# msyriac/orphics

Hardware: AMD Instinct MI355X
Metric: QE kappa reconstructions/sec on 8192^2 maps (higher is better)
Workload: dtype f64

## Files before the change

### orphics_amd/csrc/common.hpp

```cpp
#pragma once
#include <hip/hip_runtime.h>
#include <cstdio>
#include <cstring>
#include <string>
#include "../../include/orphics_amd.h"
#include "cx.hpp"

namespace oa {

std::string& last_error_ref();

inline int fail(const std::string& msg) {
    last_error_ref() = msg;
    return 1;
}

#define OA_HIP(expr)                                                                              \
    do {                                                                                          \
        hipError_t _e = (expr);                                                                   \
        if (_e != hipSuccess)                                                                     \
            return ::oa::fail(std::string(#expr) + ": " + hipGetErrorString(_e) + " (" + __FILE__ + \
                              ":" + std::to_string(__LINE__) + ")");                              \
    } while (0)

// ... 2 lines not shown
        if (!(cond)) return ::oa::fail(std::string(msg)); \
    } while (0)

#define OA_LAUNCH_CHECK() OA_HIP(hipGetLastError())

template <typename T, int N>
struct alignas(sizeof(T) * N > 16 ? 16 : sizeof(T) * N) Arr {
    T v[N];
};

struct DivBinFuse {
    const int32_t* ids; long ipitch;
    const int32_t* ids_t;
    const void* fn_t;
    int tab_logc, tab_rows;
    double pnorm; int nids, nxh;
    double* part;
    long part_cap;
    double* sums;
    unsigned* ticket;
    const int64_t* mcounts; int64_t* n; double* S; double* C;
    int store;
    int gx;
    bool done;
};

inline int flat_grid(long units, int block = 256, int cap = 8192) {
    long g = (units + block - 1) / block;
    if (g < 1) g = 1;
    if (g > cap) g = cap;
// ... 151 lines not shown
```

### orphics_amd/csrc/fft.hip

```cpp
#include <cmath>
#include <vector>
#include "fft_launch.hpp"
#include "fft_r2c_w64.hpp"
#include "fft_r2c_rs4096.hpp"
#include "fft_divbin.hpp"

namespace oa {

template <typename T, int MODE, class SEQ>
__global__ __launch_bounds__(row_maxnt<SEQ>(), waves_per_eu<T>()) void row_fft_kernel(RowArgs<T> a) {
    GpuCtx c{oa_dyn_smem};
    row_fft_body<T, MODE, SEQ>(c, a);
}

#ifndef OA_W64_OCC
#define OA_W64_OCC 1
#endif
__global__ __launch_bounds__(64, OA_W64_OCC) void row_r2c_w64_kernel(RowW64Args a) {
    GpuCtx c{oa_dyn_smem};
    row_r2c_w64_body(c, a);
}

template <typename T, class SEQ, int LR, bool PF>
__global__ __launch_bounds__(row_maxnt<SEQ>(), (sizeof(T) == 8 || PF ? 2 : 3)) void row_r2c_rsplit_kernel(RowArgs<T> a) {
// ... 117 lines not shown
    row_qe8_body<T, A, NZ, LAY, CHAIN>(c, a);
}

template <typename T, class SEQ>
__global__ __launch_bounds__(col_maxnt<SEQ>(), fused_col_waves_per_eu<T>()) void col_div_kernel(ColDivArgs<T> a) {
    GpuCtx c{oa_dyn_smem};
    col_div_body<T, SEQ>(c, a);
}

template <typename T, class SEQ, int LOGC>
__global__ __launch_bounds__((sizeof(T) == 8 ? 512 : 1024), (sizeof(T) == 8 ? 2 : 4)) void col_div_sp_kernel(ColDivArgs<T> a) {
    GpuCtx c{oa_dyn_smem};
    col_div_body<T, SEQ, GpuCtx, LOGC>(c, a);
}

template <typename T, class SEQ, int LOGC>
__global__ __launch_bounds__((sizeof(T) == 8 ? 512 : 1024), (sizeof(T) == 8 ? 2 : 4)) void col_div_sp_bin_kernel(ColDivArgs<T> a, DivBinFuse f) {
    GpuCtx c{oa_dyn_smem};
    col_div_body<T, SEQ, GpuCtx, LOGC, DivBinTail<T>>(c, a, DivBinTail<T>{f});
}

template <typename T, int LOGQ, int LOGC>
__global__ __launch_bounds__((sizeof(T) == 8 ? 384 : 768), (sizeof(T) == 8 ? 2 : 3)) void col_div3_sp_kernel(ColDivArgs<T> a) {
    GpuCtx c{oa_dyn_smem};
    col_div3_body<T, LOGQ, LOGC>(c, a);
}
template <typename T, int LOGQ, int LOGC>
__global__ __launch_bounds__((sizeof(T) == 8 ? 384 : 768), (sizeof(T) == 8 ? 2 : 3)) void col_div3_sp_bin_kernel(ColDivArgs<T> a, DivBinFuse f) {
    GpuCtx c{oa_dyn_smem};
    col_div3_body<T, LOGQ, LOGC, GpuCtx, DivBinTail<T>>(c, a, DivBinTail<T>{f});
}

template <typename T, class SEQ>
__global__ __launch_bounds__(col_maxnt<SEQ>(), waves_per_eu<T>()) void col_deriv_kernel(ColDerivArgs<T> a) {
    GpuCtx c{oa_dyn_smem};
    col_deriv_body<T, SEQ>(c, a);
}

template <typename T, class SEQ>
__global__ __launch_bounds__(col_maxnt<SEQ>(), waves_per_eu<T>()) void col_fft_kernel(ColArgs<T> a) {
    GpuCtx c{oa_dyn_smem};
    col_fft_body<T, SEQ>(c, a);
}

template <typename T, class SEQ>
// ... 274 lines not shown
        if (rc) return;
        rc = launch_col_fwdlegs_cg<T>(st, gx, gy, nt, smem, logL, a, gz);
    }
    template <typename T>
    void col_div(int gx, int gy, int nt, size_t smem, int logL, const ColDivArgs<T>& a, int gz = 1) {
        const bool ok = dispatch_seq(logL, [&](auto seq) {
            using S = decltype(seq);
            if constexpr (seq_logl<S>() <= 8) {
                if (nt > col_maxnt<S>()) { if (!rc) rc = fail("fft: column workgroup size exceeds its launch bound"); return; }
                go(col_div_kernel<T, S>, dim3(gx, gy, gz), nt, smem, a);
            } else if (!rc) rc = fail("fft: unsupported column sub-length");
        });
        if (!ok && !rc) rc = fail("fft: unsupported column length");
    }
    DivBinFuse* fuse = nullptr;
    template <class K, typename T>
    void go_fused(K kern, int gx, int gz, int nt, size_t smem, ColDivArgs<T> a) {
        {
            const hipError_t e = ensure_dyn_lds(reinterpret_cast<const void*>(kern), smem);
            if (e != hipSuccess) { rc = fail(std::string("hipFuncSetAttribute: ") + hipGetErrorString(e)); return; }
        }
        fuse->gx = gx;
        if (!fuse->store) a.out = nullptr;
        const bool tabs = fuse->tab_logc == a.logC && fuse->tab_rows == a.ny;
        a.Fn_t = (tabs && a.fn_moff == 0) ? (const T*)fuse->fn_t : nullptr;
        if (!tabs) fuse->ids_t = nullptr;
        hipLaunchKernelGGL(kern, dim3(gx, 1, gz), dim3(nt), smem, st, a, *fuse);
        hipError_t e = hipGetLastError();
        if (e != hipSuccess) rc = fail(std::string("fft launch: ") + hipGetErrorString(e));
        fuse->done = true;
    }
    template <typename T>
    bool col_div_sp(int gx, size_t smem, int logL, const ColDivArgs<T>& a, int gz = 1) {
        if (rc) return true;
        const int lt = Fft2dPlan<T>::div_lt(), nt = (1 << lt) / EPT;
        const bool narrow = lt < (sizeof(T) == 4 ? 14 : 13);
        constexpr int lc11 = sizeof(T) == 4 ? 3 : 2, lc10 = lc11 + 1;
        if (fuse && !a.accumulate && (long)gx * gz * fuse->nids <= fuse->part_cap && (logL == 10 || logL == 11 || (logL == 12 && !narrow)) &&
            (size_t)(nt / 64) * fuse->nids * sizeof(double) <= ((size_t)1 << lt) * sizeof(cx<T>)) {
            if (logL == 12) go_fused(col_div_sp_bin_kernel<T, Seq<16, 16, 16>, lc11 - 1>, gx, gz, nt, smem, a);
            else if (logL == 11 && !narrow) go_fused(col_div_sp_bin_kernel<T, Seq<16, 16, 8>, lc11>, gx, gz, nt, smem, a);
            else if (logL == 10 && !narrow) go_fused(col_div_sp_bin_kernel<T, Seq<16, 16, 4>, lc10>, gx, gz, nt, smem, a);
            else if (logL == 11) go_fused(col_div_sp_bin_kernel<T, Seq<16, 16, 8>, lc11 - 1>, gx, gz, nt, smem, a);
            else go_fused(col_div_sp_bin_kernel<T, Seq<16, 16, 4>, lc10 - 1>, gx, gz, nt, smem, a);
            return true;
        }
        if (logL == 12 && !narrow) { go(col_div_sp_kernel<T, Seq<16, 16, 16>, lc11 - 1>, dim3(gx, 1, gz), nt, smem, a); return true; }
        if (logL == 11 && !narrow) { go(col_div_sp_kernel<T, Seq<16, 16, 8>, lc11>, dim3(gx, 1, gz), nt, smem, a); return true; }
        if (logL == 10 && !narrow) { go(col_div_sp_kernel<T, Seq<16, 16, 4>, lc10>, dim3(gx, 1, gz), nt, smem, a); return true; }
        if (logL == 11) { go(col_div_sp_kernel<T, Seq<16, 16, 8>, lc11 - 1>, dim3(gx, 1, gz), nt, smem, a); return true; }
        if (logL == 10) { go(col_div_sp_kernel<T, Seq<16, 16, 4>, lc10 - 1>, dim3(gx, 1, gz), nt, smem, a); return true; }
        return false;
    }
    template <typename T>
    void col_div3(int gx, size_t smem, int rows, const ColDivArgs<T>& a, int gz = 1) {
        if (rc) return;
        constexpr int lc = sizeof(T) == 4 ? 3 : 2;
        if (rows != 1536 && rows != 768) { rc = fail("fft: unsupported 3 x 2^k divergence grid"); return; }
        const int nt = a.NT;
        if (fuse && !a.accumulate && (long)gx * gz * fuse->nids <= fuse->part_cap &&
            (size_t)(nt / 64) * fuse->nids * sizeof(double) <= ((size_t)rows << a.logC) * sizeof(cx<T>)) {
            if (rows == 1536) go_fused(col_div3_sp_bin_kernel<T, 8, lc>, gx, gz, nt, smem, a);
            else go_fused(col_div3_sp_bin_kernel<T, 7, lc + 1>, gx, gz, nt, smem, a);
            return;
        }
        if (rows == 1536) go(col_div3_sp_kernel<T, 8, lc>, dim3(gx, 1, gz), nt, smem, a);
        else go(col_div3_sp_kernel<T, 7, lc + 1>, dim3(gx, 1, gz), nt, smem, a);
    }
    template <typename T>
    void col_deriv(int gx, int gy, int nt, size_t smem, const ColDerivArgs<T>& a, int nz) {
        const bool ok = dispatch_seq(a.logL, [&](auto seq) {
            using S = decltype(seq);
            if constexpr (seq_logl<S>() <= 8) {
                if (nt > col_maxnt<S>()) { if (!rc) rc = fail("fft: column workgroup size exceeds its launch bound"); return; }
                go(col_deriv_kernel<T, S>, dim3(gx, gy, nz), nt, smem, a);
            } else if (!rc) rc = fail("fft: unsupported column sub-length");
        });
        if (!ok && !rc) rc = fail("fft: unsupported column length");
// ... 722 lines not shown
```

### orphics_amd/csrc/fft_divbin.hpp

```cpp
#pragma once
#include "fft_launch.hpp"

namespace oa {

#if defined(__HIP_DEVICE_COMPILE__) && !(defined(__gfx942__) || defined(__gfx950__))
#error "DivBinTail: the ticket hand-over relies on gfx942 / gfx950 behaviour (agent-scope relaxed atomic stores are sc1 write-through, stores count in vmcnt)"
#endif

template <int CTRL>
__device__ __forceinline__ double dpp_f64(double v) {
    const unsigned long long u = __builtin_bit_cast(unsigned long long, v);
    const int lo = __builtin_amdgcn_update_dpp(0, (int)(unsigned)u, CTRL, 0xf, 0xf, false);
    const int hi = __builtin_amdgcn_update_dpp(0, (int)(unsigned)(u >> 32), CTRL, 0xf, 0xf, false);
    return __builtin_bit_cast(double, ((unsigned long long)(unsigned)hi << 32) | (unsigned long long)(unsigned)lo);
}
__device__ __forceinline__ double readlane_f64(double v, int lane) {
    const unsigned long long u = __builtin_bit_cast(unsigned long long, v);
    const unsigned lo = (unsigned)__builtin_amdgcn_readlane((int)(unsigned)u, lane);
    const unsigned hi = (unsigned)__builtin_amdgcn_readlane((int)(unsigned)(u >> 32), lane);
    return __builtin_bit_cast(double, ((unsigned long long)hi << 32) | (unsigned long long)lo);
}
__device__ __forceinline__ double wave_total_f64(double v) {
    v += dpp_f64<0xB1>(v);
    v += dpp_f64<0x4E>(v);
    v += dpp_f64<0x141>(v);
    v += dpp_f64<0x140>(v);
    return ((readlane_f64(v, 0) + readlane_f64(v, 16)) + readlane_f64(v, 32)) + readlane_f64(v, 48);
}

template <typename T>
struct DivBinTail {
    static constexpr bool active = true;
    DivBinFuse f;
    double* rows = nullptr;

    __device__ __forceinline__ void begin(GpuCtx&, void* lds) {
        rows = reinterpret_cast<double*>(lds);
        const int nw = blockDim.x >> 6;
        for (int i = threadIdx.x; i < nw * f.nids; i += blockDim.x) rows[i] = 0.0;
    }
    __device__ __forceinline__ int id_at(unsigned yfull, int col) const { return f.ids[(long)yfull * f.ipitch + col]; }
    __device__ __forceinline__ bool packed_ids() const { return f.ids_t != nullptr; }
    __device__ __forceinline__ int id_at_t(long i) const { return f.ids_t[i]; }
    __device__ __forceinline__ void add(GpuCtx&, int id, T pw, int col) {
        const int m = (col == 0 || col == f.nxh) ? 1 : (col < f.nxh ? 2 : 0);
        const bool ok = id >= 0 && id < f.nids && m > 0;
        const double v = ok ? (double)(pw * (T)f.pnorm) * (double)m : 0.0;
        const int lane = threadIdx.x & 63;
        double* row = rows + (threadIdx.x >> 6) * f.nids;
        unsigned long long act = __ballot(ok);
        while (act) {
            const int leader = __ffsll((long long)act) - 1;
            const int lid = __shfl(id, leader, 64);
            const bool mine = ok && id == lid;
            const unsigned long long mm = __ballot(mine);
            const double sv = wave_total_f64(mine ? v : 0.0);
            if (lane == leader) row[lid] += sv;
            act &= ~mm;
        }
    }
    __device__ __forceinline__ void finish(GpuCtx&) {
        __shared__ int s_last;
        const int t = threadIdx.x, nt = blockDim.x, nw = nt >> 6, nids = f.nids;
        __syncthreads();
        const long wg = (long)blockIdx.z * gridDim.x + blockIdx.x;
        for (int i = t; i < nids; i += nt) {
            double s = 0.0;
            for (int k = 0; k < nw; ++k) s += rows[k * nids + i];
            __hip_atomic_store(f.part + wg * nids + i, s, __ATOMIC_RELAXED, __HIP_MEMORY_SCOPE_AGENT);
        }
        asm volatile("s_waitcnt vmcnt(0)" ::: "memory");
        __syncthreads();
        if (t == 0)
            s_last = (__hip_atomic_fetch_add(f.ticket, 1u, OA_TICKET_ORDER, __HIP_MEMORY_SCOPE_AGENT) == gridDim.x * gridDim.z - 1) ? 1 : 0;
        __syncthreads();
        if (!s_last) return;
        const int d = nids - 2;
        int NI = 1;
        while (NI < nids && NI < nt) NI <<= 1;
        const int G = nt / NI > 0 ? nt / NI : 1, gi = t / NI, ii = t - gi * NI;
        double* red = rows;
        const int gx = (int)gridDim.x;
        for (int z = 0; z < (int)gridDim.z; ++z) {
            for (int i0 = 0; i0 < nids; i0 += NI) {
                const int i = i0 + ii;
                __syncthreads();
                if (gi < G) {
                    double s = 0.0;
                    if (i < nids) {
                        const double* pz = f.part + ((long)z * gx) * nids + i;
                        int b = gi;
                        for (; b + 3 * G < gx; b += 4 * G) {
                            const double p0 = __hip_atomic_load(pz + (long)b * nids, __ATOMIC_RELAXED, __HIP_MEMORY_SCOPE_AGENT);
                            const double p1 = __hip_atomic_load(pz + (long)(b + G) * nids, __ATOMIC_RELAXED, __HIP_MEMORY_SCOPE_AGENT);
                            const double p2 = __hip_atomic_load(pz + (long)(b + 2 * G) * nids, __ATOMIC_RELAXED, __HIP_MEMORY_SCOPE_AGENT);
                            const double p3 = __hip_atomic_load(pz + (long)(b + 3 * G) * nids, __ATOMIC_RELAXED, __HIP_MEMORY_SCOPE_AGENT);
                            s += (p0 + p1) + (p2 + p3);
                        }
                        for (; b < gx; b += G) s += __hip_atomic_load(pz + (long)b * nids, __ATOMIC_RELAXED, __HIP_MEMORY_SCOPE_AGENT);
                    }
                    red[gi * NI + ii] = s;
                }
                __syncthreads();
                double tot = 0.0;
                if (gi == 0 && i < nids) {
                    for (int k = 0; k < G; ++k) tot += red[k * NI + ii];
                    f.sums[(long)z * nids + i] = tot;
                }
                __syncthreads();
                if (gi == 0 && i >= 1 && i <= d) red[G * NI + i - 1] = tot / (double)f.mcounts[i];
            }
            __syncthreads();
            const double* bv = red + G * NI;
            if (f.S) {
                for (int a = t; a < d; a += nt) f.S[a] += bv[a];
                for (long e = t; e < (long)d * d; e += nt) {
                    const int ra = (int)(e / d), cb = (int)(e - (long)ra * d);
                    f.C[e] += bv[ra] * bv[cb];
                }
            }
        }
        if (t == 0) {
            if (f.n) f.n[0] += (int64_t)gridDim.z;
            __hip_atomic_store(f.ticket, 0u, __ATOMIC_RELAXED, __HIP_MEMORY_SCOPE_AGENT);
        }
    }
};

}
```

### orphics_amd/csrc/fft_kernels.hpp

```cpp
#pragma once
#include <type_traits>
#include "cx.hpp"
#include "philox.hpp"

namespace oa {

constexpr int EPT = 16;
#ifndef OA_COL_LOGC
#define OA_COL_LOGC 5
#endif
constexpr int COL_LOGC = OA_COL_LOGC;

enum RowMode { ROW_R2C = 0, ROW_C2R = 1, ROW_C2C_F = 2, ROW_C2C_I = 3, ROW_WIN = 4 };

template <typename T>
OA_HD cx<T> w16(int k) {
    const T c1 = (T)0.92387953251128673848L;
    const T s1 = (T)0.38268343236508978178L;
    const T h = (T)0.70710678118654752440L;
    switch (k) {
        case 0: return mk<T>((T)1, (T)0);
        case 1: return mk<T>(c1, -s1);
        case 2: return mk<T>(h, -h);
        case 3: return mk<T>(s1, -c1);
// ... 1471 lines not shown
    long pitch;
    long opitch;
    int width, logC, NT;
    const cx<T>* tw;
    int logTw;
    long in_gs, in_ns, out_gs, out_ks;
    int accumulate;
    int rband, ny;
    int yshift;
    long in_moff, out_moff;
    long fn_moff;
    const T* Fn_t;
};

struct NoDivTail {
    static constexpr bool active = false;
    template <class Ctx> OA_HD void begin(Ctx&, void*) {}
    OA_HD int id_at(unsigned, int) const { return -1; }
    OA_HD bool packed_ids() const { return false; }
    OA_HD int id_at_t(long) const { return -1; }
    template <class Ctx, typename T> OA_HD void add(Ctx&, int, T, int) {}
    template <class Ctx> OA_HD void finish(Ctx&) {}
};

template <typename T, class SEQ, class Ctx, int LOGC = COL_LOGC, class Tail = NoDivTail>
OA_HD void col_div_body(Ctx& ctx, const ColDivArgs<T>& a, Tail tail = Tail{}) {
    cx<T>* s = reinterpret_cast<cx<T>*>(ctx.smem());
    constexpr int logL = Log2x<SEQ::r0>::v + Log2x<SEQ::r1>::v + Log2x<SEQ::r2>::v + Log2x<SEQ::r3>::v;
    constexpr int n = SEQ::n;
    constexpr int RL = SEQ::get(n - 1), LRL = Log2x<RL>::v, NB = EPT / RL;
    constexpr int logNs = logL - LRL;
    constexpr int logC = LOGC;
    constexpr int NT = ((1 << (seq_total_log<SEQ>() + LOGC)) / EPT) > 0 ? ((1 << (seq_total_log<SEQ>() + LOGC)) / EPT) : 1;
    const int tid = ctx.tid();
    int tile = ctx.bid_x();
    if ((sizeof(cx<T>) << LOGC) < 128) {
// ... 23 lines not shown
        ctx.sync();
        stage_out<T, R0, false, false>(s, vb, tid, NT, logL, logC, 0, 0, NoStore{});
        ctx.sync();
        stage_in<T, RL, false, false>(s, vb, tid, NT, logL, logC, 0, l0, twl, logL, NoLoad{});
    } else {
        col_pipeline_to_regs<T, SEQ>(ctx, s, va, tid, NT, logC, twl, logL, la);
        ctx.sync();
        col_pipeline_to_regs<T, SEQ>(ctx, s, vb, tid, NT, logC, twl, logL, lb);
    }
    const long oorg = g * a.out_gs * a.opitch + c0;
    const T* Fnb = a.Fn + zmap * a.fn_moff + oorg;
    cx<T>* outb = a.out + omo + oorg;
    const unsigned ostr = (unsigned)(a.out_ks * a.opitch);
    if constexpr (Tail::active) {
        ctx.sync();
        tail.begin(ctx, s);
        ctx.sync();
        T pw[EPT];
        int idv[EPT];
#pragma unroll
        for (int u = 0; u < NB; ++u) {
            const int b = tid + u * NT;
            const int c = b & ((1 << logC) - 1), j = b >> logC;
            const bool cok = c < ncols;
            const int kq = j & ((1 << logNs) - 1);
            const int base = ((j - kq) << LRL) + kq;
            const T lx = cok ? a.lxd[c0 + c] : (T)0;
#pragma unroll
            for (int t = 0; t < RL; ++t) {
                const int k = base + (t << logNs);
                const unsigned y = (unsigned)(g * a.out_gs) + (unsigned)k * (unsigned)a.out_ks;
                const bool ok = cok && !(a.rband && (int)y >= a.rband && (int)y <= a.ny - a.rband);
                const unsigned up = (a.yshift && y >= (unsigned)(a.ny >> 1)) ? (unsigned)a.yshift : 0u;
                const unsigned i = (unsigned)k * ostr + (unsigned)c + up * (unsigned)a.opitch;
                pw[u * RL + t] = (T)0;
                idv[u * RL + t] = -1;
                if (ok) {
                    const long ti_ = (((long)tile << logL) + k) * (1 << logC) + c;
                    const T fn = a.Fn_t ? a.Fn_t[ti_] : Fnb[i];
                    cx<T> d = mul_pi(va[u * RL + t] * lx + vb[u * RL + t] * a.lyd[y + up]) * fn;
                    if (a.out) {
                        if (a.accumulate) d = d + outb[i];
                        outb[i] = d;
                    }
                    pw[u * RL + t] = d.x * d.x + d.y * d.y;
                    idv[u * RL + t] = tail.packed_ids() ? tail.id_at_t((((long)tile << logL) + k) * (1 << logC) + c) : tail.id_at(y + up, c0 + c);
                }
            }
        }
#pragma unroll
        for (int u = 0; u < NB; ++u) {
            const int c = (tid + u * NT) & ((1 << logC) - 1);
#pragma unroll
            for (int t = 0; t < RL; ++t) tail.add(ctx, idv[u * RL + t], pw[u * RL + t], c0 + c);
        }
        tail.finish(ctx);
    } else {
#pragma unroll
    for (int u = 0; u < NB; ++u) {
        const int b = tid + u * NT;
        const int c = b & ((1 << logC) - 1), j = b >> logC;
        if (c >= ncols) continue;
        const int kq = j & ((1 << logNs) - 1);
        const int base = ((j - kq) << LRL) + kq;
        const T lx = a.lxd[c0 + c];
#pragma unroll
        for (int t = 0; t < RL; ++t) {
            const int k = base + (t << logNs);
            const unsigned y = (unsigned)(g * a.out_gs) + (unsigned)k * (unsigned)a.out_ks;
// ... 74 lines not shown
#pragma unroll
            for (int r = 0; r < 6; ++r) x[it][r] = s[((r * Q + pk[it]) << logC) + pc[it]];
            const cx<T> w3 = w1[it] * w2[it], w5 = w4[it] * w1[it];
            x[it][1] = x[it][1] * w1[it]; x[it][2] = x[it][2] * w2[it]; x[it][3] = x[it][3] * w3;
            x[it][4] = x[it][4] * w4[it]; x[it][5] = x[it][5] * w5;
            dft6<T>(x[it]);
        }
    };
    finish(va, xa);
    ctx.sync();
    finish(vb, xb);
    const T* Fnb = a.Fn + zmap * a.fn_moff + c0;
    cx<T>* outb = a.out + omo + c0;
    if constexpr (Tail::active) {
        ctx.sync();
        tail.begin(ctx, s);
        ctx.sync();
        T pw[NIT * 6];
        int idv[NIT * 6];
#pragma unroll
        for (int it = 0; it < NIT; ++it) {
            const int c = pc[it], k = pk[it];
            const bool cok = pv[it] && c < ncols;
            const T lx = cok ? a.lxd[c0 + c] : (T)0;
#pragma unroll
            for (int q = 0; q < 6; ++q) {
                const unsigned y = (unsigned)(k + Q * q);
                const bool ok = cok && !(a.rband && (int)y >= a.rband && (int)y <= a.ny - a.rband);
                const unsigned up = (a.yshift && y >= (unsigned)(N >> 1)) ? (unsigned)a.yshift : 0u;
                const unsigned i = (y + up) * (unsigned)a.opitch + (unsigned)c;
                pw[it * 6 + q] = (T)0;
                idv[it * 6 + q] = -1;
                if (ok) {
                    const long ti_ = ((long)tile * N + y) * C + c;
                    const T fn = a.Fn_t ? a.Fn_t[ti_] : Fnb[i];
                    cx<T> d = mul_pi(xa[it][q] * lx + xb[it][q] * a.lyd[y + up]) * fn;
                    if (a.out) {
                        if (a.accumulate) d = d + outb[i];
                        outb[i] = d;
                    }
                    pw[it * 6 + q] = d.x * d.x + d.y * d.y;
                    idv[it * 6 + q] = tail.packed_ids() ? tail.id_at_t(ti_) : tail.id_at(y + up, c0 + c);
                }
            }
        }
#pragma unroll
        for (int it = 0; it < NIT; ++it) {
#pragma unroll
            for (int q = 0; q < 6; ++q) tail.add(ctx, idv[it * 6 + q], pw[it * 6 + q], c0 + pc[it]);
        }
        tail.finish(ctx);
    } else {
#pragma unroll
        for (int it = 0; it < NIT; ++it) {
            const int c = pc[it], k = pk[it];
            if (!pv[it] || c >= ncols) continue;
            const T lx = a.lxd[c0 + c];
#pragma unroll
            for (int q = 0; q < 6; ++q) {
                const unsigned y = (unsigned)(k + Q * q);
                if (a.rband && (int)y >= a.rband && (int)y <= a.ny - a.rband) continue;
                const unsigned up = (a.yshift && y >= (unsigned)(N >> 1)) ? (unsigned)a.yshift : 0u;
                const unsigned i = (y + up) * (unsigned)a.opitch + (unsigned)c;
                cx<T> d = mul_pi(xa[it][q] * lx + xb[it][q] * a.lyd[y + up]) * Fnb[i];
// ... 442 lines not shown
```

### orphics_amd/csrc/pipeline.hip

```cpp
#include <dlfcn.h>
#include <cstdlib>
#include <algorithm>
#include <functional>
#include <string>
#include <utility>
#include <vector>
#include "common.hpp"
#include "fft_plan.hpp"

namespace oa {

constexpr int MC_BATCH_MAX = 6;

struct DevBuf {
    void* p = nullptr;
    size_t bytes = 0;
    int reserve(size_t need, bool zero = false) {
        if (bytes >= need) return 0;
        if (p) { OA_HIP(hipDeviceSynchronize()); release(); }
        OA_HIP(hipMalloc(&p, need));
        bytes = need;
        if (zero) OA_HIP(hipMemset(p, 0, need));
        return 0;
    }
// ... 32 lines not shown
    DevBuf rdn0_pool;
    unsigned long rdn0_gen = 0;
    int rdn0_my = 0;
    int rdn0_ran_batched = 0;
    DevBuf rdn0mv_legs;
    DevBuf rdn0mv_pool;
    DevBuf n1_pool;
    std::vector<const void*> rdn0mv_key;
    int rdn0mv_band[5] = {0, 0, 0, 0, 0};
    int rdn0mv_my = 0;
    unsigned long rdn0mv_gen = 0;
    struct DivTabs {
        DevBuf fn_t, ids_t;
        unsigned long tab_gen = 0;
        int tab_rows = 0, tab_logc = 0, tab_wk = 0;
    } dt[2];
    DivTabs& tabs_of(int rows) { return (my3 && rows == my3) ? dt[1] : dt[0]; }
    const DivTabs& tabs_of(int rows) const { return (my3 && rows == my3) ? dt[1] : dt[0]; }
    unsigned long bind_gen = 1;
    DevBuf fb_t;
    unsigned long fb_gen = 0;
    int fb_my = 0, fb_wl = 0, fb_rl = 0;
    void** mv_ftab = nullptr;
    std::vector<const void*> mv_fkey;
    int opt_mc_batch = MC_BATCH_MAX;
    bool opt_mv_batch = true;
    bool opt_mv_rowbatch = true;
    bool opt_mv_chain = true;
    bool opt_divbin = true;
    bool opt_win_fused = true;
// ... 50 lines not shown
    return 0;
}

void pipeline_release(oa_plan* p) {
    if (!p || !p->pipe) return;
    Pipeline* q = (Pipeline*)p->pipe;
    if (q->work) (void)hipFree(q->work);
    if (q->bin_scratch) (void)hipFree(q->bin_scratch);
    if (q->sums) (void)hipFree(q->sums);
    if (q->counts_full) (void)hipFree(q->counts_full);
    if (q->counts_tmp) (void)hipFree(q->counts_tmp);
    if (q->ticket) (void)hipFree(q->ticket);
    if (q->mv_ftab) (void)hipFree(q->mv_ftab);
    if (q->mv_rtab) (void)hipFree(q->mv_rtab);
    for (DevBuf* b : {&q->split_legs, &q->mc_src, &q->lens_pool, &q->mvmc, &q->mvwin, &q->rdn0_legs, &q->rdn0_pool, &q->rdn0mv_legs, &q->rdn0mv_pool, &q->n1_pool, &q->dt[0].fn_t, &q->dt[0].ids_t,
                      &q->dt[1].fn_t, &q->dt[1].ids_t, &q->fb_t}) b->release();
    if (q->band) (void)oa_plan_destroy(q->band);
    q->release_band();
    q->brows.release();
    q->bs_tab.release();
    if (q->pb.plan) (void)oa_plan_destroy(q->pb.plan);
    for (DevBuf* b : {&q->pb.planes, &q->pb.stab, &q->pb.mrows, &q->pb.mwin, &q->pb.mc.pool}) b->release();
    delete q;
    p->pipe = nullptr;
}

static int ensure_work(oa_plan* p, Pipeline* q) {
    if (q->work) return 0;
    const size_t pb = plane_bytes(p);
    OA_HIP(hipMalloc(&q->work, 7 * pb));
    OA_HIP(hipMemset(q->work, 0, 7 * pb));
// ... 233 lines not shown
                                                nullptr, q->bin_scratch, 0, 0, stream)
                                 : fail(std::string("oa_plan_set_bins: padded bin ids: ") + hipGetErrorString(e));
        (void)hipStreamSynchronize((hipStream_t)stream);
        (void)hipFree(ids4);
        if (z4) (void)hipFree(z4);
        if (rc) return rc;
    }
    if (p->mixed) return (q->FG && q->band) ? mixed_bins(p, q, (hipStream_t)stream) : 0;
    return ensure_div_tables(p, q, (hipStream_t)stream);
}

void* oa_plan_kappa(oa_plan* p) { return (p && p->pipe) ? ((Pipeline*)p->pipe)->kk : nullptr; }
const int64_t* oa_plan_bin_counts(oa_plan* p) { return (p && p->pipe) ? ((Pipeline*)p->pipe)->counts_full : nullptr; }

static bool divbin_enabled(const Pipeline* q) { return q->opt_divbin; }
static int ensure_div_tables(oa_plan* p, Pipeline* q, hipStream_t st, int rows) {
    Pipeline::DivTabs* const t = &q->tabs_of(rows);
    if (!(q->Fn && q->ids && (rows == 1024 || rows == 2048 || rows == 4096 || (q->my3 && rows == q->my3)) && q->wk > 0)) { t->tab_rows = 0; return 0; }
    const int logc = div_tile_logc(p, rows);
    if (t->tab_gen == q->bind_gen && t->tab_rows == rows && t->tab_logc == logc && t->tab_wk == q->wk) return 0;
    const size_t rs = p->dtype == OA_F32 ? 4 : 8;
    const long tiles = ((long)q->wk + (1 << logc) - 1) >> logc, total = (tiles * rows) << logc;
    if (int rc = t->fn_t.reserve((size_t)total * rs)) return rc;
    if (int rc = t->ids_t.reserve((size_t)total * 4)) return rc;
    if (int rc = pack_tiles(p, q->Fn, t->fn_t.p, rows, logc, q->wk, (int)rs, st)) return rc;
    if (int rc = pack_tiles(p, q->ids, t->ids_t.p, rows, logc, q->wk, 4, st)) return rc;
    t->tab_gen = q->bind_gen; t->tab_rows = rows; t->tab_logc = logc; t->tab_wk = q->wk;
    return 0;
}
static int ensure_div_tables(oa_plan* p, Pipeline* q, hipStream_t st) {
    if (int rc = ensure_div_tables(p, q, st, q->my)) return rc;
    return q->my3 ? ensure_div_tables(p, q, st, q->my3) : 0;
}
static const void* fband_table(oa_plan* p, Pipeline* q, hipStream_t st) {
    static const bool off = exp_env("OA_NO_FBAND_TABLE") != nullptr;
    const int my = q->map_grid();
    if (off || !q->FG || my <= 0 || !qe_rsplit_lr(p, my, q->wl, q->wk, q->mrow)) return nullptr;
    if (q->fb_t.p && q->fb_gen == q->bind_gen && q->fb_my == my && q->fb_wl == q->wl && q->fb_rl == q->rl) return q->fb_t.p;
    if (q->fb_t.reserve((size_t)qe_fband_table_entries(p, q->wl, my) * elem_bytes(p))) { (void)hipGetLastError(); return nullptr; }
    if (qe_fband_pack_w(p, q->FG, q->FH, q->fb_t.p, q->wl, q->rl, my, st)) return nullptr;
    q->fb_gen = q->bind_gen; q->fb_my = my; q->fb_wl = q->wl; q->fb_rl = q->rl;
    return q->fb_t.p;
}
static DivBinFuse make_fuse(const oa_plan* p, const Pipeline* q, int64_t* n, double* S, double* C, int store, int rows = -1) {
    DivBinFuse f{};
    if (rows < 0) rows = q->my;
    const Pipeline::DivTabs& t = q->tabs_of(rows);
    if (t.tab_rows && t.tab_gen == q->bind_gen && t.tab_rows == rows && t.tab_wk == q->wk) {
        f.ids_t = (const int32_t*)t.ids_t.p; f.fn_t = t.fn_t.p; f.tab_logc = t.tab_logc; f.tab_rows = t.tab_rows;
    }
    f.ids = q->ids; f.ipitch = p->kp; f.pnorm = q->norm; f.nids = q->nids; f.nxh = p->nx / 2;
    f.part = (double*)q->bin_scratch; f.part_cap = (long)(oa_bin_scratch_bytes(q->nids) / (long)sizeof(double)) * MC_BATCH_MAX;
    f.sums = q->sums; f.ticket = q->ticket; f.mcounts = q->counts_full; f.n = n; f.S = S; f.C = C; f.store = store; f.done = false;
    return f;
}

static int qe_tt_impl(oa_plan* p, const void* real_map, const void* kX, const void* kY, void* out_kappa_hc, int zero_outside,
                      void* stream, DivBinFuse* fuse, int rows_done = 0);
static int qe_mv_pow2(oa_plan* p, Pipeline* q, const MvCall& c, void* out, int accumulate, int leg_cols, int kappa_cols, int leg_rows,
                      int kappa_rows, int mrow, int zero_outside, hipStream_t st, bool keep_planes);
int oa_qe_tt(oa_plan* p, const void* real_map, const void* kX, const void* kY, void* out_kappa_hc, int zero_outside,
             void* stream) {
    if (p && p->mixed) {
        OA_REQUIRE(p->pipe && ((Pipeline*)p->pipe)->FG, "oa_qe_tt: call oa_plan_set_filters first");
// ... 2014 lines not shown
```

Measured before the change: 5971.

## Bin fused column power via precomputed per-tile run-length tables of bin ids

Builds a host-side table of runs of equal bin ids per column tile and uploads it. When the table is present, the fused column-divergence/binning kernel writes power into LDS by position and sums contiguous runs per bin, instead of loading per-element ids and scattering into per-wave bin rows. The aim is to remove the per-element id loads and the scattered LDS accumulation. In exchange the kernel needs more LDS, and table construction adds a blocking device-to-host copy, a host pass and stream syncs whenever the tables are rebuilt.

```diff
diff --git a/orphics_amd/csrc/common.hpp b/orphics_amd/csrc/common.hpp
--- a/orphics_amd/csrc/common.hpp
+++ b/orphics_amd/csrc/common.hpp
@@ -40,6 +40,8 @@
     const int32_t* ids_t;
     const void* fn_t;
     int tab_logc, tab_rows;
+    const unsigned long long* run_ent; const int32_t* run_off;
+    int run_w, run_rb, run_cap;
     double pnorm; int nids, nxh;
     double* part;
     long part_cap;
diff --git a/orphics_amd/csrc/divbin_runs.hpp b/orphics_amd/csrc/divbin_runs.hpp
--- /dev/null
+++ b/orphics_amd/csrc/divbin_runs.hpp
@@ -0,0 +1,65 @@
+#pragma once
+#include <cstddef>
+#include <cstdint>
+#include <vector>
+
+namespace oa {
+
+constexpr int DIVRUN_MAX_LEN = 64;
+
+inline uint64_t divrun_pack(int col, int first, int len, int id) {
+    return (uint64_t)((uint32_t)first | ((uint32_t)len << 16) | ((uint32_t)col << 24)) | ((uint64_t)(uint32_t)id << 32);
+}
+inline int divrun_first(uint64_t e) { return (int)(e & 0xffffu); }
+inline int divrun_len(uint64_t e) { return (int)((e >> 16) & 0xffu); }
+inline int divrun_col(uint64_t e) { return (int)((e >> 24) & 0xffu); }
+inline int divrun_id(uint64_t e) { return (int)(uint32_t)(e >> 32); }
+
+struct DivRunTable {
+    std::vector<uint64_t> ent;
+    std::vector<int32_t> off;
+};
+
+inline bool divbin_build_runs(const int32_t* ids_t, int tiles, int rows, int logc, int width, int rband, int nids, int nxh, int max_entries,
+                              DivRunTable* out) {
+    out->ent.clear();
+    out->off.clear();
+    if (tiles < 1 || rows < 1 || rows > 0x10000 || logc < 0 || logc > 8 || nids < 1) return false;
+    const int C = 1 << logc;
+    out->off.reserve((size_t)tiles * (nids + 1));
+    std::vector<uint64_t> runs;
+    std::vector<int32_t> cnt((size_t)nids + 1);
+    for (int t = 0; t < tiles; ++t) {
+        runs.clear();
+        const int32_t* tid = ids_t + (size_t)t * rows * C;
+        for (int c = 0; c < C; ++c) {
+            const long col = (long)t * C + c;
+            if (col >= width || col > nxh) continue;
+            int first = 0, len = 0, cur = -1;
+            for (int y = 0; y <= rows; ++y) {
+                const bool kept = y < rows && !(rband > 0 && y >= rband && y <= rows - rband);
+                const int id = kept ? tid[(size_t)y * C + c] : -1;
+                const bool valid = id >= 0 && id < nids;
+                if (len > 0 && valid && id == cur && len < DIVRUN_MAX_LEN) { ++len; continue; }
+                if (len > 0) runs.push_back(divrun_pack(c, first, len, cur));
+                len = 0;
+                if (valid) { first = y; len = 1; cur = id; }
+            }
+        }
+        if ((long)runs.size() > (long)max_entries) {
+            out->ent.clear();
+            out->off.clear();
+            return false;
+        }
+        for (int i = 0; i <= nids; ++i) cnt[i] = 0;
+        for (uint64_t e : runs) ++cnt[divrun_id(e) + 1];
+        const int32_t base = (int32_t)out->ent.size();
+        for (int i = 0; i < nids; ++i) cnt[i + 1] += cnt[i];
+        for (int i = 0; i <= nids; ++i) out->off.push_back(base + cnt[i]);
+        out->ent.resize((size_t)base + runs.size());
+        for (uint64_t e : runs) out->ent[(size_t)base + cnt[divrun_id(e)]++] = e;
+    }
+    return true;
+}
+
+}
diff --git a/orphics_amd/csrc/fft.hip b/orphics_amd/csrc/fft.hip
--- a/orphics_amd/csrc/fft.hip
+++ b/orphics_amd/csrc/fft.hip
@@ -1,3 +1,4 @@
+#include <algorithm>
 #include <cmath>
 #include <vector>
 #include "fft_launch.hpp"
@@ -155,10 +156,11 @@
     col_div_body<T, SEQ, GpuCtx, LOGC>(c, a);
 }
 
-template <typename T, class SEQ, int LOGC>
+template <typename T, bool RUNS> using DivTailOf = std::conditional_t<RUNS, DivRunTail<T>, DivBinTail<T>>;
+template <typename T, class SEQ, int LOGC, bool RUNS>
 __global__ __launch_bounds__((sizeof(T) == 8 ? 512 : 1024), (sizeof(T) == 8 ? 2 : 4)) void col_div_sp_bin_kernel(ColDivArgs<T> a, DivBinFuse f) {
     GpuCtx c{oa_dyn_smem};
-    col_div_body<T, SEQ, GpuCtx, LOGC, DivBinTail<T>>(c, a, DivBinTail<T>{f});
+    col_div_body<T, SEQ, GpuCtx, LOGC, DivTailOf<T, RUNS>>(c, a, DivTailOf<T, RUNS>{f});
 }
 
 template <typename T, int LOGQ, int LOGC>
@@ -166,10 +168,10 @@
     GpuCtx c{oa_dyn_smem};
     col_div3_body<T, LOGQ, LOGC>(c, a);
 }
-template <typename T, int LOGQ, int LOGC>
+template <typename T, int LOGQ, int LOGC, bool RUNS>
 __global__ __launch_bounds__((sizeof(T) == 8 ? 384 : 768), (sizeof(T) == 8 ? 2 : 3)) void col_div3_sp_bin_kernel(ColDivArgs<T> a, DivBinFuse f) {
     GpuCtx c{oa_dyn_smem};
-    col_div3_body<T, LOGQ, LOGC, GpuCtx, DivBinTail<T>>(c, a, DivBinTail<T>{f});
+    col_div3_body<T, LOGQ, LOGC, GpuCtx, DivTailOf<T, RUNS>>(c, a, DivTailOf<T, RUNS>{f});
 }
 
 template <typename T, class SEQ>
@@ -474,15 +476,19 @@
         if (!ok && !rc) rc = fail("fft: unsupported column length");
     }
     DivBinFuse* fuse = nullptr;
+#define OA_GO_FUSED(K, ...) go_fused(K<__VA_ARGS__, false>, K<__VA_ARGS__, true>, gx, gz, nt, smem, a)
     template <class K, typename T>
-    void go_fused(K kern, int gx, int gz, int nt, size_t smem, ColDivArgs<T> a) {
+    void go_fused(K kern_ids, K kern_runs, int gx, int gz, int nt, size_t smem, ColDivArgs<T> a) {
+        const bool tabs = fuse->tab_logc == a.logC && fuse->tab_rows == a.ny;
+        const bool runs = tabs && fuse->run_ent && fuse->run_w == a.width && fuse->run_rb == a.rband && fuse->run_cap <= 2 * nt;
+        const K kern = runs ? kern_runs : kern_ids;
+        if (runs) smem = std::max(smem, divrun_lds_bytes(a.ny, a.logC, nt, sizeof(T) == 8));
         {
             const hipError_t e = ensure_dyn_lds(reinterpret_cast<const void*>(kern), smem);
             if (e != hipSuccess) { rc = fail(std::string("hipFuncSetAttribute: ") + hipGetErrorString(e)); return; }
         }
         fuse->gx = gx;
         if (!fuse->store) a.out = nullptr;
-        const bool tabs = fuse->tab_logc == a.logC && fuse->tab_rows == a.ny;
         a.Fn_t = (tabs && a.fn_moff == 0) ? (const T*)fuse->fn_t : nullptr;
         if (!tabs) fuse->ids_t = nullptr;
         hipLaunchKernelGGL(kern, dim3(gx, 1, gz), dim3(nt), smem, st, a, *fuse);
@@ -498,11 +504,11 @@
         constexpr int lc11 = sizeof(T) == 4 ? 3 : 2, lc10 = lc11 + 1;
         if (fuse && !a.accumulate && (long)gx * gz * fuse->nids <= fuse->part_cap && (logL == 10 || logL == 11 || (logL == 12 && !narrow)) &&
             (size_t)(nt / 64) * fuse->nids * sizeof(double) <= ((size_t)1 << lt) * sizeof(cx<T>)) {
-            if (logL == 12) go_fused(col_div_sp_bin_kernel<T, Seq<16, 16, 16>, lc11 - 1>, gx, gz, nt, smem, a);
-            else if (logL == 11 && !narrow) go_fused(col_div_sp_bin_kernel<T, Seq<16, 16, 8>, lc11>, gx, gz, nt, smem, a);
-            else if (logL == 10 && !narrow) go_fused(col_div_sp_bin_kernel<T, Seq<16, 16, 4>, lc10>, gx, gz, nt, smem, a);
-            else if (logL == 11) go_fused(col_div_sp_bin_kernel<T, Seq<16, 16, 8>, lc11 - 1>, gx, gz, nt, smem, a);
-            else go_fused(col_div_sp_bin_kernel<T, Seq<16, 16, 4>, lc10 - 1>, gx, gz, nt, smem, a);
+            if (logL == 12) OA_GO_FUSED(col_div_sp_bin_kernel, T, Seq<16, 16, 16>, lc11 - 1);
+            else if (logL == 11 && !narrow) OA_GO_FUSED(col_div_sp_bin_kernel, T, Seq<16, 16, 8>, lc11);
+            else if (logL == 10 && !narrow) OA_GO_FUSED(col_div_sp_bin_kernel, T, Seq<16, 16, 4>, lc10);
+            else if (logL == 11) OA_GO_FUSED(col_div_sp_bin_kernel, T, Seq<16, 16, 8>, lc11 - 1);
+            else OA_GO_FUSED(col_div_sp_bin_kernel, T, Seq<16, 16, 4>, lc10 - 1);
             return true;
         }
         if (logL == 12 && !narrow) { go(col_div_sp_kernel<T, Seq<16, 16, 16>, lc11 - 1>, dim3(gx, 1, gz), nt, smem, a); return true; }
@@ -520,8 +526,8 @@
         const int nt = a.NT;
         if (fuse && !a.accumulate && (long)gx * gz * fuse->nids <= fuse->part_cap &&
             (size_t)(nt / 64) * fuse->nids * sizeof(double) <= ((size_t)rows << a.logC) * sizeof(cx<T>)) {
-            if (rows == 1536) go_fused(col_div3_sp_bin_kernel<T, 8, lc>, gx, gz, nt, smem, a);
-            else go_fused(col_div3_sp_bin_kernel<T, 7, lc + 1>, gx, gz, nt, smem, a);
+            if (rows == 1536) OA_GO_FUSED(col_div3_sp_bin_kernel, T, 8, lc);
+            else OA_GO_FUSED(col_div3_sp_bin_kernel, T, 7, lc + 1);
             return;
         }
         if (rows == 1536) go(col_div3_sp_kernel<T, 8, lc>, dim3(gx, 1, gz), nt, smem, a);
diff --git a/orphics_amd/csrc/fft_divbin.hpp b/orphics_amd/csrc/fft_divbin.hpp
--- a/orphics_amd/csrc/fft_divbin.hpp
+++ b/orphics_amd/csrc/fft_divbin.hpp
@@ -28,13 +28,78 @@
     return ((readlane_f64(v, 0) + readlane_f64(v, 16)) + readlane_f64(v, 32)) + readlane_f64(v, 48);
 }
 
+template <class Partial>
+__device__ __forceinline__ void divbin_handover(const DivBinFuse& f, double* red, Partial partial) {
+    __shared__ int s_last;
+    const int t = threadIdx.x, nt = blockDim.x, nids = f.nids;
+    const long wg = (long)blockIdx.z * gridDim.x + blockIdx.x;
+    for (int i = t; i < nids; i += nt) {
+        const double s = partial(i);
+        __hip_atomic_store(f.part + wg * nids + i, s, __ATOMIC_RELAXED, __HIP_MEMORY_SCOPE_AGENT);
+    }
+    asm volatile("s_waitcnt vmcnt(0)" ::: "memory");
+    __syncthreads();
+    if (t == 0)
+        s_last = (__hip_atomic_fetch_add(f.ticket, 1u, OA_TICKET_ORDER, __HIP_MEMORY_SCOPE_AGENT) == gridDim.x * gridDim.z - 1) ? 1 : 0;
+    __syncthreads();
+    if (!s_last) return;
+    const int d = nids - 2;
+    int NI = 1;
+    while (NI < nids && NI < nt) NI <<= 1;
+    const int G = nt / NI > 0 ? nt / NI : 1, gi = t / NI, ii = t - gi * NI;
+    const int gx = (int)gridDim.x;
+    for (int z = 0; z < (int)gridDim.z; ++z) {
+        for (int i0 = 0; i0 < nids; i0 += NI) {
+            const int i = i0 + ii;
+            __syncthreads();
+            if (gi < G) {
+                double s = 0.0;
+                if (i < nids) {
+                    const double* pz = f.part + ((long)z * gx) * nids + i;
+                    int b = gi;
+                    for (; b + 3 * G < gx; b += 4 * G) {
+                        const double p0 = __hip_atomic_load(pz + (long)b * nids, __ATOMIC_RELAXED, __HIP_MEMORY_SCOPE_AGENT);
+                        const double p1 = __hip_atomic_load(pz + (long)(b + G) * nids, __ATOMIC_RELAXED, __HIP_MEMORY_SCOPE_AGENT);
+                        const double p2 = __hip_atomic_load(pz + (long)(b + 2 * G) * nids, __ATOMIC_RELAXED, __HIP_MEMORY_SCOPE_AGENT);
+                        const double p3 = __hip_atomic_load(pz + (long)(b + 3 * G) * nids, __ATOMIC_RELAXED, __HIP_MEMORY_SCOPE_AGENT);
+                        s += (p0 + p1) + (p2 + p3);
+                    }
+                    for (; b < gx; b += G) s += __hip_atomic_load(pz + (long)b * nids, __ATOMIC_RELAXED, __HIP_MEMORY_SCOPE_AGENT);
+                }
+                red[gi * NI + ii] = s;
+            }
+            __syncthreads();
+            double tot = 0.0;
+            if (gi == 0 && i < nids) {
+                for (int k = 0; k < G; ++k) tot += red[k * NI + ii];
+                f.sums[(long)z * nids + i] = tot;
+            }
+            __syncthreads();
+            if (gi == 0 && i >= 1 && i <= d) red[G * NI + i - 1] = tot / (double)f.mcounts[i];
+        }
+        __syncthreads();
+        const double* bv = red + G * NI;
+        if (f.S) {
+            for (int a = t; a < d; a += nt) f.S[a] += bv[a];
+            for (long e = t; e < (long)d * d; e += nt) {
+                const int ra = (int)(e / d), cb = (int)(e - (long)ra * d);
+                f.C[e] += bv[ra] * bv[cb];
+            }
+        }
+    }
+    if (t == 0) {
+        if (f.n) f.n[0] += (int64_t)gridDim.z;
+        __hip_atomic_store(f.ticket, 0u, __ATOMIC_RELAXED, __HIP_MEMORY_SCOPE_AGENT);
+    }
+}
+
 template <typename T>
 struct DivBinTail {
-    static constexpr bool active = true;
+    static constexpr bool active = true, needs_ids = true;
     DivBinFuse f;
     double* rows = nullptr;
 
-    __device__ __forceinline__ void begin(GpuCtx&, void* lds) {
+    __device__ __forceinline__ void begin(GpuCtx&, void* lds, int, int, int) {
         rows = reinterpret_cast<double*>(lds);
         const int nw = blockDim.x >> 6;
         for (int i = threadIdx.x; i < nw * f.nids; i += blockDim.x) rows[i] = 0.0;
@@ -42,7 +107,7 @@
     __device__ __forceinline__ int id_at(unsigned yfull, int col) const { return f.ids[(long)yfull * f.ipitch + col]; }
     __device__ __forceinline__ bool packed_ids() const { return f.ids_t != nullptr; }
     __device__ __forceinline__ int id_at_t(long i) const { return f.ids_t[i]; }
-    __device__ __forceinline__ void add(GpuCtx&, int id, T pw, int col) {
+    __device__ __forceinline__ void add(GpuCtx&, int id, T pw, int col, int) {
         const int m = (col == 0 || col == f.nxh) ? 1 : (col < f.nxh ? 2 : 0);
         const bool ok = id >= 0 && id < f.nids && m > 0;
         const double v = ok ? (double)(pw * (T)f.pnorm) * (double)m : 0.0;
@@ -60,71 +125,87 @@
         }
     }
     __device__ __forceinline__ void finish(GpuCtx&) {
-        __shared__ int s_last;
-        const int t = threadIdx.x, nt = blockDim.x, nw = nt >> 6, nids = f.nids;
-        __syncthreads();
-        const long wg = (long)blockIdx.z * gridDim.x + blockIdx.x;
-        for (int i = t; i < nids; i += nt) {
+        const int nw = blockDim.x >> 6, nids = f.nids;
+        const double* r = rows;
+        __syncthreads();
+        divbin_handover(f, rows, [=](int i) {
             double s = 0.0;
-            for (int k = 0; k < nw; ++k) s += rows[k * nids + i];
-            __hip_atomic_store(f.part + wg * nids + i, s, __ATOMIC_RELAXED, __HIP_MEMORY_SCOPE_AGENT);
-        }
-        asm volatile("s_waitcnt vmcnt(0)" ::: "memory");
-        __syncthreads();
-        if (t == 0)
-            s_last = (__hip_atomic_fetch_add(f.ticket, 1u, OA_TICKET_ORDER, __HIP_MEMORY_SCOPE_AGENT) == gridDim.x * gridDim.z - 1) ? 1 : 0;
-        __syncthreads();
-        if (!s_last) return;
-        const int d = nids - 2;
-        int NI = 1;
-        while (NI < nids && NI < nt) NI <<= 1;
-        const int G = nt / NI > 0 ? nt / NI : 1, gi = t / NI, ii = t - gi * NI;
-        double* red = rows;
-        const int gx = (int)gridDim.x;
-        for (int z = 0; z < (int)gridDim.z; ++z) {
-            for (int i0 = 0; i0 < nids; i0 += NI) {
-                const int i = i0 + ii;
-                __syncthreads();
-                if (gi < G) {
-                    double s = 0.0;
-                    if (i < nids) {
-                        const double* pz = f.part + ((long)z * gx) * nids + i;
-                        int b = gi;
-                        for (; b + 3 * G < gx; b += 4 * G) {
-                            const double p0 = __hip_atomic_load(pz + (long)b * nids, __ATOMIC_RELAXED, __HIP_MEMORY_SCOPE_AGENT);
-                            const double p1 = __hip_atomic_load(pz + (long)(b + G) * nids, __ATOMIC_RELAXED, __HIP_MEMORY_SCOPE_AGENT);
-                            const double p2 = __hip_atomic_load(pz + (long)(b + 2 * G) * nids, __ATOMIC_RELAXED, __HIP_MEMORY_SCOPE_AGENT);
-                            const double p3 = __hip_atomic_load(pz + (long)(b + 3 * G) * nids, __ATOMIC_RELAXED, __HIP_MEMORY_SCOPE_AGENT);
-                            s += (p0 + p1) + (p2 + p3);
-                        }
-                        for (; b < gx; b += G) s += __hip_atomic_load(pz + (long)b * nids, __ATOMIC_RELAXED, __HIP_MEMORY_SCOPE_AGENT);
-                    }
-                    red[gi * NI + ii] = s;
-                }
-                __syncthreads();
-                double tot = 0.0;
-                if (gi == 0 && i < nids) {
-                    for (int k = 0; k < G; ++k) tot += red[k * NI + ii];
-                    f.sums[(long)z * nids + i] = tot;
-                }
-                __syncthreads();
-                if (gi == 0 && i >= 1 && i <= d) red[G * NI + i - 1] = tot / (double)f.mcounts[i];
-            }
-            __syncthreads();
-            const double* bv = red + G * NI;
-            if (f.S) {
-                for (int a = t; a < d; a += nt) f.S[a] += bv[a];
-                for (long e = t; e < (long)d * d; e += nt) {
-                    const int ra = (int)(e / d), cb = (int)(e - (long)ra * d);
-                    f.C[e] += bv[ra] * bv[cb];
-                }
-            }
-        }
-        if (t == 0) {
-            if (f.n) f.n[0] += (int64_t)gridDim.z;
-            __hip_atomic_store(f.ticket, 0u, __ATOMIC_RELAXED, __HIP_MEMORY_SCOPE_AGENT);
-        }
+            for (int k = 0; k < nw; ++k) s += r[k * nids + i];
+            return s;
+        });
     }
 };
 
-}
+__host__ __device__ inline int divrun_col_stride(int rows, int logc) {
+    const int want = (32 >> logc) > 0 ? (32 >> logc) : 1;
+    const int s = rows + (rows >> 6) + 1;
+    return s + (((want - s) % 32) + 32) % 32;
+}
+inline size_t divrun_lds_bytes(int rows, int logc, int nt, bool f64) {
+    return ((size_t)divrun_col_stride(rows, logc) << logc) * sizeof(double) + (f64 ? (size_t)2 * nt * sizeof(double) : 0);
+}
+template <typename T>
+struct DivRunTail {
+    static constexpr bool active = true, needs_ids = false;
+    static constexpr bool r_behind = sizeof(T) == 8;
+    DivBinFuse f;
+    double* P = nullptr;
+    double* R = nullptr;
+    const int32_t* offp = nullptr;
+    int base = 0, cnt = 0, logc = 0, cs = 0, o0 = 0, o1 = 0;
+    unsigned e0 = 0, e1 = 0;
+
+    __device__ __forceinline__ void begin(GpuCtx&, void* lds, int tile, int logc_, int rows) {
+        P = reinterpret_cast<double*>(lds);
+        logc = logc_;
+        cs = divrun_col_stride(rows, logc);
+        R = r_behind ? P + ((long)cs << logc) : P;
+        const int t = threadIdx.x, nt = blockDim.x;
+        const int32_t* off = offp = f.run_off + (long)tile * (f.nids + 1);
+        base = off[0];
+        cnt = off[f.nids] - base;
+        if (cnt > 2 * nt) cnt = 2 * nt;
+        const unsigned* ew = reinterpret_cast<const unsigned*>(f.run_ent + base);
+        e0 = t < cnt ? ew[2 * t] : 0u;
+        e1 = t + nt < cnt ? ew[2 * (t + nt)] : 0u;
+        if (t < f.nids) { o0 = off[t] - base; o1 = off[t + 1] - base; }
+    }
+    __device__ __forceinline__ int id_at(unsigned, int) const { return -1; }
+    __device__ __forceinline__ bool packed_ids() const { return false; }
+    __device__ __forceinline__ int id_at_t(long) const { return -1; }
+    __device__ __forceinline__ void add(GpuCtx&, int, T pw, int col, int slot) {
+        const int m = (col == 0 || col == f.nxh) ? 1 : (col < f.nxh ? 2 : 0);
+        const int y = slot >> logc, c = slot & ((1 << logc) - 1);
+        P[c * cs + y + (y >> 6)] = (double)(pw * (T)f.pnorm) * (double)m;
+    }
+    __device__ __forceinline__ double run_sum(unsigned w) const {
+        const int first = (int)(w & 0xffffu), len = (int)((w >> 16) & 0xffu), col = (int)(w >> 24);
+        const double* p = P + col * cs;
+        double s = 0.0;
+#pragma unroll 4
+        for (int y = first; y < first + len; ++y) s += p[y + (y >> 6)];
+        return s;
+    }
+    __device__ __forceinline__ void finish(GpuCtx&) {
+        const int t = threadIdx.x, nt = blockDim.x;
+        __syncthreads();
+        const double s0 = run_sum(e0), s1 = run_sum(e1);
+        if (!r_behind) __syncthreads();
+        if (t < cnt) R[t] = s0;
+        if (t + nt < cnt) R[t + nt] = s1;
+        __syncthreads();
+        const double* r = R;
+        const int32_t* off = offp;
+        const int a0 = o0, a1 = o1, b0 = base, n = cnt;
+        divbin_handover(f, P, [=](int i) {
+            int k = a0, k1 = a1;
+            if (i != t) { k = off[i] - b0; k1 = off[i + 1] - b0; }
+            if (k1 > n) k1 = n;
+            double s = 0.0;
+            for (; k < k1; ++k) s += r[k];
+            return s;
+        });
+    }
+};
+
+}
diff --git a/orphics_amd/csrc/fft_kernels.hpp b/orphics_amd/csrc/fft_kernels.hpp
--- a/orphics_amd/csrc/fft_kernels.hpp
+++ b/orphics_amd/csrc/fft_kernels.hpp
@@ -1509,12 +1509,12 @@
 };
 
 struct NoDivTail {
-    static constexpr bool active = false;
-    template <class Ctx> OA_HD void begin(Ctx&, void*) {}
+    static constexpr bool active = false, needs_ids = false;
+    template <class Ctx> OA_HD void begin(Ctx&, void*, int, int, int) {}
     OA_HD int id_at(unsigned, int) const { return -1; }
     OA_HD bool packed_ids() const { return false; }
     OA_HD int id_at_t(long) const { return -1; }
-    template <class Ctx, typename T> OA_HD void add(Ctx&, int, T, int) {}
+    template <class Ctx, typename T> OA_HD void add(Ctx&, int, T, int, int) {}
     template <class Ctx> OA_HD void finish(Ctx&) {}
 };
 
@@ -1568,7 +1568,7 @@
     const unsigned ostr = (unsigned)(a.out_ks * a.opitch);
     if constexpr (Tail::active) {
         ctx.sync();
-        tail.begin(ctx, s);
+        tail.begin(ctx, s, tile, logC, 1 << logL);
         ctx.sync();
         T pw[EPT];
         int idv[EPT];
@@ -1598,15 +1598,19 @@
                         outb[i] = d;
                     }
                     pw[u * RL + t] = d.x * d.x + d.y * d.y;
-                    idv[u * RL + t] = tail.packed_ids() ? tail.id_at_t((((long)tile << logL) + k) * (1 << logC) + c) : tail.id_at(y + up, c0 + c);
+                    if constexpr (Tail::needs_ids)
+                        idv[u * RL + t] = tail.packed_ids() ? tail.id_at_t((((long)tile << logL) + k) * (1 << logC) + c) : tail.id_at(y + up, c0 + c);
+                    else tail.add(ctx, 0, d.x * d.x + d.y * d.y, c0 + c, (k << logC) + c);
                 }
             }
         }
-#pragma unroll
-        for (int u = 0; u < NB; ++u) {
-            const int c = (tid + u * NT) & ((1 << logC) - 1);
-#pragma unroll
-            for (int t = 0; t < RL; ++t) tail.add(ctx, idv[u * RL + t], pw[u * RL + t], c0 + c);
+        if constexpr (Tail::needs_ids) {
+#pragma unroll
+            for (int u = 0; u < NB; ++u) {
+                const int c = (tid + u * NT) & ((1 << logC) - 1);
+#pragma unroll
+                for (int t = 0; t < RL; ++t) tail.add(ctx, idv[u * RL + t], pw[u * RL + t], c0 + c, -1);
+            }
         }
         tail.finish(ctx);
     } else {
@@ -1711,7 +1715,7 @@
     cx<T>* outb = a.out + omo + c0;
     if constexpr (Tail::active) {
         ctx.sync();
-        tail.begin(ctx, s);
+        tail.begin(ctx, s, tile, logC, N);
         ctx.sync();
         T pw[NIT * 6];
         int idv[NIT * 6];
@@ -1737,14 +1741,17 @@
                         outb[i] = d;
                     }
                     pw[it * 6 + q] = d.x * d.x + d.y * d.y;
-                    idv[it * 6 + q] = tail.packed_ids() ? tail.id_at_t(ti_) : tail.id_at(y + up, c0 + c);
+                    if constexpr (Tail::needs_ids) idv[it * 6 + q] = tail.packed_ids() ? tail.id_at_t(ti_) : tail.id_at(y + up, c0 + c);
+                    else tail.add(ctx, 0, d.x * d.x + d.y * d.y, c0 + c, (int)(y << logC) + c);
                 }
             }
         }
-#pragma unroll
-        for (int it = 0; it < NIT; ++it) {
-#pragma unroll
-            for (int q = 0; q < 6; ++q) tail.add(ctx, idv[it * 6 + q], pw[it * 6 + q], c0 + pc[it]);
+        if constexpr (Tail::needs_ids) {
+#pragma unroll
+            for (int it = 0; it < NIT; ++it) {
+#pragma unroll
+                for (int q = 0; q < 6; ++q) tail.add(ctx, idv[it * 6 + q], pw[it * 6 + q], c0 + pc[it], -1);
+            }
         }
         tail.finish(ctx);
     } else {
diff --git a/orphics_amd/csrc/pipeline.hip b/orphics_amd/csrc/pipeline.hip
--- a/orphics_amd/csrc/pipeline.hip
+++ b/orphics_amd/csrc/pipeline.hip
@@ -7,6 +7,7 @@
 #include <vector>
 #include "common.hpp"
 #include "fft_plan.hpp"
+#include "divbin_runs.hpp"
 
 namespace oa {
 
@@ -70,6 +71,9 @@
         DevBuf fn_t, ids_t;
         unsigned long tab_gen = 0;
         int tab_rows = 0, tab_logc = 0, tab_wk = 0;
+        DevBuf run_ent, run_off;
+        bool has_runs = false;
+        int run_w = 0, run_rb = 0, run_cap = 0;
     } dt[2];
     DivTabs& tabs_of(int rows) { return (my3 && rows == my3) ? dt[1] : dt[0]; }
     const DivTabs& tabs_of(int rows) const { return (my3 && rows == my3) ? dt[1] : dt[0]; }
@@ -150,7 +154,7 @@
     if (q->mv_ftab) (void)hipFree(q->mv_ftab);
     if (q->mv_rtab) (void)hipFree(q->mv_rtab);
     for (DevBuf* b : {&q->split_legs, &q->mc_src, &q->lens_pool, &q->mvmc, &q->mvwin, &q->rdn0_legs, &q->rdn0_pool, &q->rdn0mv_legs, &q->rdn0mv_pool, &q->n1_pool, &q->dt[0].fn_t, &q->dt[0].ids_t,
-                      &q->dt[1].fn_t, &q->dt[1].ids_t, &q->fb_t}) b->release();
+                      &q->dt[1].fn_t, &q->dt[1].ids_t, &q->dt[0].run_ent, &q->dt[0].run_off, &q->dt[1].run_ent, &q->dt[1].run_off, &q->fb_t}) b->release();
     if (q->band) (void)oa_plan_destroy(q->band);
     q->release_band();
     q->brows.release();
@@ -414,6 +418,25 @@
 const int64_t* oa_plan_bin_counts(oa_plan* p) { return (p && p->pipe) ? ((Pipeline*)p->pipe)->counts_full : nullptr; }
 
 static bool divbin_enabled(const Pipeline* q) { return q->opt_divbin; }
+static int build_run_table(const oa_plan* p, Pipeline* q, Pipeline::DivTabs* t, int rows, int logc, long tiles, hipStream_t st) {
+    t->has_runs = false;
+    const int nxh = p->nx / 2;
+    const int w = q->wk > nxh + 1 ? nxh + 1 : q->wk;
+    const int rb = (q->rk <= 0 || 2L * q->rk - 1 >= rows) ? 0 : q->rk;
+    const int cap = 2 * ((rows << logc) / 16);
+    std::vector<int32_t> host((size_t)(tiles * rows) << logc);
+    OA_HIP(hipMemcpyAsync(host.data(), t->ids_t.p, host.size() * 4, hipMemcpyDeviceToHost, st));
+    OA_HIP(hipStreamSynchronize(st));
+    DivRunTable tab;
+    if (!divbin_build_runs(host.data(), (int)tiles, rows, logc, w, rb, q->nids, nxh, cap, &tab)) return 0;
+    if (int rc = t->run_ent.reserve((tab.ent.size() + 1) * 8)) return rc;
+    if (int rc = t->run_off.reserve(tab.off.size() * 4)) return rc;
+    OA_HIP(hipMemcpyAsync(t->run_ent.p, tab.ent.data(), tab.ent.size() * 8, hipMemcpyHostToDevice, st));
+    OA_HIP(hipMemcpyAsync(t->run_off.p, tab.off.data(), tab.off.size() * 4, hipMemcpyHostToDevice, st));
+    OA_HIP(hipStreamSynchronize(st));
+    t->has_runs = true; t->run_w = w; t->run_rb = rb; t->run_cap = cap;
+    return 0;
+}
 static int ensure_div_tables(oa_plan* p, Pipeline* q, hipStream_t st, int rows) {
     Pipeline::DivTabs* const t = &q->tabs_of(rows);
     if (!(q->Fn && q->ids && (rows == 1024 || rows == 2048 || rows == 4096 || (q->my3 && rows == q->my3)) && q->wk > 0)) { t->tab_rows = 0; return 0; }
@@ -425,6 +448,7 @@
     if (int rc = t->ids_t.reserve((size_t)total * 4)) return rc;
     if (int rc = pack_tiles(p, q->Fn, t->fn_t.p, rows, logc, q->wk, (int)rs, st)) return rc;
     if (int rc = pack_tiles(p, q->ids, t->ids_t.p, rows, logc, q->wk, 4, st)) return rc;
+    if (int rc = build_run_table(p, q, t, rows, logc, tiles, st)) return rc;
     t->tab_gen = q->bind_gen; t->tab_rows = rows; t->tab_logc = logc; t->tab_wk = q->wk;
     return 0;
 }
@@ -448,6 +472,10 @@
     const Pipeline::DivTabs& t = q->tabs_of(rows);
     if (t.tab_rows && t.tab_gen == q->bind_gen && t.tab_rows == rows && t.tab_wk == q->wk) {
         f.ids_t = (const int32_t*)t.ids_t.p; f.fn_t = t.fn_t.p; f.tab_logc = t.tab_logc; f.tab_rows = t.tab_rows;
+        if (t.has_runs) {
+            f.run_ent = (const unsigned long long*)t.run_ent.p; f.run_off = (const int32_t*)t.run_off.p;
+            f.run_w = t.run_w; f.run_rb = t.run_rb; f.run_cap = t.run_cap;
+        }
     }
     f.ids = q->ids; f.ipitch = p->kp; f.pnorm = q->norm; f.nids = q->nids; f.nxh = p->nx / 2;
     f.part = (double*)q->bin_scratch; f.part_cap = (long)(oa_bin_scratch_bytes(q->nids) / (long)sizeof(double)) * MC_BATCH_MAX;
```

Measured after the change: 6048, median of 6. 1.3% higher.
